# yzqin/s4g-release

Measured on AMD Instinct MI355X. Metric: scenes/sec (25.6k-pt clouds) end-to-end grasp inference, higher is better.
Workload: dtype f32 (f16x2 split)

## Files before the change

include/s4g_ops.h:

```cpp
#ifndef S4G_OPS_H_
#define S4G_OPS_H_

#include <stddef.h>
#include <stdint.h>

#ifdef __cplusplus
extern "C" {
#endif

#define S4G_ABI_VERSION 14


#define S4G_OK 0
#define S4G_EINVAL (-1)
#define S4G_EWORKSPACE (-2)
#define S4G_EUNSUPPORTED (-3)

#define S4G_FLAG_FMAD 1

typedef void *s4g_stream_t;

#define S4G_OP_FPS 1
#define S4G_OP_BALL_QUERY 2
#define S4G_OP_THREE_NN 3
// ... 131 lines not shown
  float *out2;
  int32_t ldc2, split_n;
  float *out_amax2;
  int32_t a_L;
} s4g_gemm_desc_t;

int s4g_mlp_gemm_f32(const s4g_gemm_desc_t *desc, s4g_stream_t stream);

typedef struct s4g_heads_desc {
  int32_t precision, P, N, ldx;
  int32_t C, H0, H1, H2, H3;
  const float *X;
  const void *W_frag[5];
  const float *bias[5];
  const float *w_inv_scale[5];
  float *out[4];
  int32_t channels[4];
  int32_t sigmoid_head;
  const float *a_amax;
  float a_amax_floor;
  int32_t rows_per_scene;
  const void *pre_W_frag[2];
  const float *pre_bias[2];
  const float *pre_w_inv_scale[2];
  const int32_t *pre_nidx;
  const float *pre_nw;
  const float *pre_sparse;
  const float *pre_dense;
  const float *pre_lbias;
  const float *pre_a_amax2;
  int32_t pre_N2;
  int64_t out_batch_stride;
  int32_t head_mask;
} s4g_heads_desc_t;

int s4g_heads_chain_f32(const s4g_heads_desc_t *desc, s4g_stream_t stream);

int s4g_amax_per_scene_f32(const float *x, int64_t B, int64_t n_per_scene, float *out_slots, s4g_stream_t stream);

int s4g_gemm_chain_supported(int loader, int epilogue, int C, int Kpad16);

int s4g_ball_query_i32(const float *xyz_b3n, const float *ctr_b3m, int64_t B,
                       int64_t N, int64_t M, float radius, int64_t K,
                       int32_t *idx_bmk, int32_t *cnt_bm, void *ws,
                       size_t ws_bytes, int flags, s4g_stream_t stream);
int s4g_three_nn_weights_i32(const float *q_b3n1, const float *k_b3n2, int64_t B,
                             int64_t N1, int64_t N2, float eps, int32_t *idx_bn3,
                             float *w_bn3, void *ws, size_t ws_bytes, int flags,
                             s4g_stream_t stream);
size_t s4g_three_nn_grid_workspace_bytes(int64_t B, int64_t N1, int64_t N2);
size_t s4g_three_nn_grid_header_offset(int64_t B, int64_t N2);
int s4g_three_nn_weights_grid_i32(const float *q_b3n1, const float *k_b3n2, int64_t B,
                                  int64_t N1, int64_t N2, float eps, float cell,
                                  int32_t *idx_bn3, float *w_bn3, void *ws,
                                  size_t ws_bytes, int flags, s4g_stream_t stream);

int s4g_three_nn_grid_f32(const float *q_b3n1, const float *k_b3n2, int64_t B, int64_t N1,
                          int64_t N2, float cell, int64_t *idx_bn3, float *d2_bn3, void *ws,
                          size_t ws_bytes, int flags, s4g_stream_t stream);

int s4g_query_group_f32(const float *xyz_b3n, const float *ctr_b3m, int64_t B,
                        int64_t N, int64_t M, float radius, int64_t K,
                        int64_t *idx_bmk, int64_t *cnt_bm, float *grouped_b3mk,
                        void *ws, size_t ws_bytes, int flags, s4g_stream_t stream);

int s4g_group_rel_xyz_i32(const float *xyz_b3n, const float *ctr_b3m, const int32_t *idx_bmk,
// ... 161 lines not shown
```

s4g_release_amd/_cabi.py:

```python
import ctypes
import os

_HERE = os.path.dirname(os.path.abspath(__file__))
LIB_PATH = os.environ.get("S4G_HIP_LIB") or os.path.join(_HERE, "libs4g_hip.so")

S4G_ABI_VERSION = 14
S4G_EINVAL = -1
S4G_EWORKSPACE = -2
S4G_EUNSUPPORTED = -3
S4G_FLAG_FMAD = 1
S4G_OP_FPS, S4G_OP_BALL_QUERY, S4G_OP_THREE_NN = 1, 2, 3

_vp = ctypes.c_void_p
_i64 = ctypes.c_int64
_sz = ctypes.c_size_t
_int = ctypes.c_int
_f32 = ctypes.c_float

_i32 = ctypes.c_int32


class GemmDesc(ctypes.Structure):
    _fields_ = [
        ("loader", _i32), ("epilogue", _i32), ("groups", _i32), ("relu", _i32),
        ("P", _i32), ("Cin", _i32), ("Kpad", _i32), ("Cout", _i32),
        ("W", _vp), ("bias", _vp), ("w_gstride", _i32), ("b_gstride", _i32),
        ("A", _vp), ("lda", _i32), ("a_coff", _i32), ("a_gcol", _i32),
        ("gidx", _vp), ("feat", _vp), ("xyz", _vp), ("ctr", _vp),
        ("Cf", _i32), ("N", _i32), ("M", _i32), ("K", _i32),
        ("nidx", _vp), ("nw", _vp), ("sparse", _vp), ("dense", _vp),
        ("C2", _i32), ("C1", _i32), ("N2", _i32), ("N1", _i32),
        ("out", _vp), ("ldc", _i32), ("c_coff", _i32), ("c_gcol", _i32),
        ("cf_ptr", _vp * 4), ("cf_start", _i32 * 5), ("cf_sigmoid_from", _i32), ("cf_N", _i32),
        ("precision", _i32), ("Kpad16", _i32), ("W_bf16x3", _vp), ("mlp1_w", _vp),
        ("W_f16x2", _vp), ("w_inv_scale", _vp), ("a_amax", _vp), ("a_amax2", _vp),
        ("a_amax_floor", _f32), ("out_amax", _vp), ("W_f16x2_frag", _vp),
        ("W2_f16x2_frag", _vp), ("w2_inv_scale", _vp), ("bias2", _vp), ("Cout2", _i32), ("relu2", _i32),
        ("W3_f16x2_frag", _vp), ("w3_inv_scale", _vp), ("bias3", _vp), ("Cout3", _i32), ("relu3", _i32),
        ("loader_bias", _vp), ("rows_per_scene", _i32), ("rel_xyz4", _vp), ("seg4", _vp), ("seg_rows", _vp),
        ("out2", _vp), ("ldc2", _i32), ("split_n", _i32), ("out_amax2", _vp),
        ("a_L", _i32),
    ]


class HeadsDesc(ctypes.Structure):
    _fields_ = [
        ("precision", _i32), ("P", _i32), ("N", _i32), ("ldx", _i32),
        ("C", _i32), ("H0", _i32), ("H1", _i32), ("H2", _i32), ("H3", _i32),
        ("X", _vp), ("W_frag", _vp * 5), ("bias", _vp * 5), ("w_inv_scale", _vp * 5),
        ("out", _vp * 4), ("channels", _i32 * 4), ("sigmoid_head", _i32),
        ("a_amax", _vp), ("a_amax_floor", _f32), ("rows_per_scene", _i32),
        ("pre_W_frag", _vp * 2), ("pre_bias", _vp * 2), ("pre_w_inv_scale", _vp * 2),
        ("pre_nidx", _vp), ("pre_nw", _vp), ("pre_sparse", _vp), ("pre_dense", _vp),
        ("pre_lbias", _vp), ("pre_a_amax2", _vp), ("pre_N2", _i32), ("out_batch_stride", _i64), ("head_mask", _i32),
    ]


SIGNATURES = {
    "s4g_mlp_gemm_f32": (_int, [ctypes.POINTER(GemmDesc), _vp]),
    "s4g_heads_chain_f32": (_int, [ctypes.POINTER(HeadsDesc), _vp]),
    "s4g_ball_query_i32": (_int, [_vp, _vp, _i64, _i64, _i64, _f32, _i64, _vp, _vp, _vp, _sz,
                                  _int, _vp]),
    "s4g_three_nn_weights_i32": (_int, [_vp, _vp, _i64, _i64, _i64, _f32, _vp, _vp, _vp, _sz,
                                        _int, _vp]),
    "s4g_three_nn_grid_workspace_bytes": (_sz, [_i64, _i64, _i64]),
    "s4g_three_nn_grid_header_offset": (_sz, [_i64, _i64]),
    "s4g_three_nn_weights_grid_i32": (_int, [_vp, _vp, _i64, _i64, _i64, _f32, _f32, _vp, _vp, _vp,
                                             _sz, _int, _vp]),
    "s4g_three_nn_grid_f32": (_int, [_vp, _vp, _i64, _i64, _i64, _f32, _vp, _vp, _vp, _sz, _int, _vp]),
    "s4g_group_points_xyz_f32": (_int, [_vp, _vp, _i64, _i64, _i64, _i64, _vp, _vp, _sz, _vp]),
    "s4g_gemm_chain_supported": (_int, [_int, _int, _int, _int]),
    "s4g_amax_per_scene_f32": (_int, [_vp, _i64, _i64, _vp, _vp]),
    "s4g_interp_add_cl_f32": (_int, [_vp, _vp, _vp, _vp, _vp, _i64, _i64, _i64, _i64, _int, _vp, _vp, _vp]),
    "s4g_group_points_ws_f32": (_int, [_vp, _vp, _i64, _i64, _i64, _i64, _i64, _vp, _vp, _sz, _vp]),
    "s4g_three_interpolate_ws_f32": (_int, [_vp, _vp, _vp, _i64, _i64, _i64, _i64, _vp, _vp, _sz, _int, _vp]),
    "s4g_fps_gather_i32": (_int, [_vp, _i64, _i64, _i64, _vp, _vp, _vp, _sz, _int, _vp]),
    "s4g_fps_prepass_f32": (_int, [_vp, _i64, _i64, _i64, _vp, _vp, _vp]),
    "s4g_fps_gather_ex_i32": (_int, [_vp, _i64, _i64, _i64, _vp, _vp, _vp, _vp, _vp, _sz, _int, _vp]),
    "s4g_fps_prefix_check_f32": (_int, [_vp, _vp, _i64, _i64, _i64, _vp, _int, _vp]),
    "s4g_build_variants": (_int, []),
    "s4g_test_knobs_enabled": (_int, []),
    "s4g_fps_f64": (_int, [_vp, _i64, _i64, _i64, _vp, _vp, _sz, _int, _vp]),
    "s4g_ball_query_f64": (_int, [_vp, _vp, _i64, _i64, _i64, _f32, _i64, _vp, _vp, _int, _vp]),
    "s4g_three_nn_f64": (_int, [_vp, _vp, _i64, _i64, _i64, _vp, _vp, _int, _vp]),
    "s4g_group_points_f64": (_int, [_vp, _vp, _i64, _i64, _i64, _i64, _i64, _vp, _vp]),
    "s4g_group_points_backward_f64": (_int, [_vp, _vp, _i64, _i64, _i64, _i64, _i64, _vp, _vp]),
    "s4g_three_interpolate_f64": (_int, [_vp, _vp, _vp, _i64, _i64, _i64, _i64, _vp, _int, _vp]),
# ... 120 lines not shown
```

s4g_release_amd/csrc/mlp_heads.hip:

```cpp
#include <stdlib.h>

#include "mlp_common.h"

#ifndef S4G_HEADS_ABLATE
#define S4G_HEADS_ABLATE 0
#endif

namespace s4g {

__device__ __forceinline__ void heads_keep_alive(const f32x16& v) { asm volatile("" ::"v"(v)); }

struct HeadsParams {
  int P, N;
  const float* X;
  int ldx;
  const uint16_t* W[5];
  const float* bias[5];
  const float* wsc[5];
  float* out[4];
  int ch[4];
  long long obs[4];
  int head_mask;
  int sigmoid_head;
  const float* a_amax;
  float a_floor;
  int rps;
  const uint16_t* Wp[2];
  const float* bias_p[2];
  const float* wsc_p[2];
  const int* nidx;
  const float* nw;
  const float* sparse;
  const float* dense;
  const float* lbias;
  const float* a_amax2;
  int N2;
};

template <int PL, int HD_RING, int NRBT, bool PRE>
__global__ __launch_bounds__(512, 2) void mlp_heads_kernel(const HeadsParams p) {
  constexpr int BM = 32 * NRBT, C = 256, NW = 8, astr = C + 8, aplane = BM * astr;
  constexpr int FB = PL * 1024;
  extern __shared__ __attribute__((aligned(16))) float smemf[];
  uint16_t* PA = reinterpret_cast<uint16_t*>(smemf);
  uint16_t* PB = PA + PL * aplane;
  float* scr = reinterpret_cast<float*>(PB + PL * aplane);

  const int t = threadIdx.x;
  const int lane = t & 63;
  const int li = lane & 31, lh = lane >> 5;
  const int wv = __builtin_amdgcn_readfirstlane(t >> 6);
  const int p0 = blockIdx.x * BM;
  const uint32_t wf_lane = (uint32_t)lane * 16u;

  float sa = 1.f, inv_sa = 1.f;
  if constexpr (PL == 2) {
    float amax = p.a_floor;
    if constexpr (PRE) {
      if (p.a_amax) amax += amax_rows(p.a_amax, lane, p0, min(p0 + BM, p.P) - 1, p.rps);
      if (p.a_amax2) amax += amax_rows(p.a_amax2, lane, p0, min(p0 + BM, p.P) - 1, p.rps);
    } else if (p.a_amax) {
      amax = fmaxf(amax, amax_rows(p.a_amax, lane, p0, min(p0 + BM, p.P) - 1, p.rps));
    }
    uint32_t ex = __float_as_uint(amax) >> 23;
    ex = ex < 15u ? 15u : (ex > 240u ? 240u : ex);
    ex = __builtin_amdgcn_readfirstlane(ex);
    sa = __uint_as_float((268u - ex) << 23);
    inv_sa = __uint_as_float((ex - 14u) << 23);
  }

  WRef wrs[5];
#pragma unroll
  for (int L = 0; L < 5; ++L) wrs[L] = wref(p.W[L], 0);
  auto woff = [&](int n32, int nks, int ks) { return (size_t)((n32 * nks + ks) * FB); };
  auto w0 = [&](int g, int h) { return wrs[0] + woff(g * 16 + h * 8 + wv, 16, 0); };
  auto w1 = [&](int g, int h) { return wrs[1] + woff(g * 8 + wv, 32, h * 16); };
  auto w2 = [&](int g) { return wrs[2] + woff(g * 8 + wv, 16, 0); };
  auto w3 = [&](int g) { return wrs[3] + woff(g * 4 + (wv & 3), 16, 0); };
  auto wl = [&](int g) { return wrs[4] + woff(g, 8, 0); };
  auto wload = [&](const WRef& w, uint32_t byte_off, int pl) { return wref_load(w, wf_lane + pl * 1024, byte_off); };
  const WRef wp0 = PRE ? wref(p.Wp[0], woff(wv, 16, 0)) : wrs[0];
  const WRef wp1 = PRE ? wref(p.Wp[1], woff(wv, 16, 0)) : wrs[0];

  const int hmask = p.head_mask;
  const int g_first = __builtin_ctz(hmask);
  uint4 ring[HD_RING][PL];
  {
    const WRef w = PRE ? wp0 : w0(g_first, 0);
#pragma unroll
    for (int d = 0; d < HD_RING; ++d)
#pragma unroll
      for (int pl = 0; pl < PL; ++pl) ring[d][pl] = wload(w, d * FB, pl);
  }

#pragma unroll 1
  for (int r0 = 0; r0 < BM; r0 += 64) {
    const int row = r0 + (t >> 3), chunk = t & 7;
    const bool ok = p0 + row < p.P;
    float4 ra[8];
    if constexpr (PRE) {
      const int pos = ok ? p0 + row : 0;
      const int bq = pos / p.N;
      int i3[3];
      float w3[3];
#pragma unroll
      for (int k = 0; k < 3; ++k) {
        i3[k] = bq * p.N2 + p.nidx[(size_t)pos * 3 + k];
        w3[k] = p.nw[(size_t)pos * 3 + k];
      }
#pragma unroll
      for (int h = 0; h < 2; ++h) {
        float4 a[4], b[4], c[4], y[4], bb[4];
#pragma unroll
        for (int kk = 0; kk < 4; ++kk) {
          const int col = (h * 4 + kk) * 32 + chunk * 4;
          a[kk] = *reinterpret_cast<const float4*>(p.sparse + (size_t)i3[0] * 256 + col);
          b[kk] = *reinterpret_cast<const float4*>(p.sparse + (size_t)i3[1] * 256 + col);
          c[kk] = *reinterpret_cast<const float4*>(p.sparse + (size_t)i3[2] * 256 + col);
          bb[kk] = *reinterpret_cast<const float4*>(p.lbias + col);
          y[kk] = p.dense ? *reinterpret_cast<const float4*>(p.dense + (size_t)pos * 256 + col)
                          : make_float4(0.f, 0.f, 0.f, 0.f);
        }
#pragma unroll
        for (int kk = 0; kk < 4; ++kk) {
          const float av[4] = {a[kk].x, a[kk].y, a[kk].z, a[kk].w}, bv[4] = {b[kk].x, b[kk].y, b[kk].z, b[kk].w};
          const float cv[4] = {c[kk].x, c[kk].y, c[kk].z, c[kk].w}, yv[4] = {y[kk].x, y[kk].y, y[kk].z, y[kk].w};
          const float bi[4] = {bb[kk].x, bb[kk].y, bb[kk].z, bb[kk].w};
          float r[4];
#pragma unroll
          for (int e = 0; e < 4; ++e) {
            float acc = __fmul_rn(av[e], w3[0]);
            acc = __fadd_rn(acc, __fmul_rn(bv[e], w3[1]));
            acc = __fadd_rn(acc, __fmul_rn(cv[e], w3[2]));
            r[e] = ok ? fmaxf(__fadd_rn(__fadd_rn(yv[e], acc), bi[e]), 0.f) : 0.f;
          }
          ra[h * 4 + kk] = make_float4(r[0], r[1], r[2], r[3]);
        }
      }
    } else {
    const float* src = p.X + (size_t)(ok ? p0 + row : 0) * p.ldx + chunk * 4;
#pragma unroll
    for (int kt = 0; kt < 8; ++kt)
      ra[kt] = ok ? nt_load4(src + kt * 32) : make_float4(0.f, 0.f, 0.f, 0.f);
    }
#pragma unroll
    for (int kt = 0; kt < 8; ++kt) {
      uint16_t* dst = PA + row * astr + kt * 32 + chunk * 4;
      if constexpr (PL == 2) {
        uint2 h, l;
        split2_h<false>(ra[kt], sa, h, l);
        *reinterpret_cast<uint2*>(dst) = h;
        *reinterpret_cast<uint2*>(dst + aplane) = l;
      } else {
        *reinterpret_cast<uint2*>(dst) = make_uint2(cvt_pk_bf16(ra[kt].x, ra[kt].y), cvt_pk_bf16(ra[kt].z, ra[kt].w));
      }
    }
  }
  __syncthreads();

#define S4G_HD_TERM(NRB, PA_, PB_, ZERO)                                                            \
  _Pragma("unroll") for (int rb = 0; rb < NRB; ++rb)                                                \
    acc[rb] = chain_mfma<PL>(bf[PB_], af[rb][PA_], (ZERO) ? zero16 : acc[rb]);
#define S4G_HD_STRIP(PANEL, NRB, ROWOFF, WCUR, NKS, WNEXT)                                          \
  {                                                                                                 \
    const uint16_t* a_lane = (PANEL) + ((ROWOFF) + li) * astr + 8 * lh;                             \
    uint4 afn[NRBT][PL];                                                                            \
    _Pragma("unroll") for (int rb = 0; rb < NRB; ++rb) _Pragma("unroll") for (int pl = 0; pl < PL; ++pl) \
      afn[rb][pl] = *reinterpret_cast<const uint4*>(a_lane + pl * aplane + rb * 32 * astr);         \
    const WRef wcur_ = (WCUR);                                                                      \
    const WRef wnext_ = (WNEXT);                                                                    \
    _Pragma("unroll") for (int ks = 0; ks < NKS; ++ks) {                                            \
      const int d = ks % HD_RING;                                                                   \
      const int ksn = ks + 1 == NKS ? 0 : ks + 1;                                                   \
      uint4 af[NRBT][PL], bf[PL];                                                                   \
      _Pragma("unroll") for (int rb = 0; rb < NRB; ++rb) _Pragma("unroll") for (int pl = 0; pl < PL; ++pl) { \
        af[rb][pl] = afn[rb][pl];                                                                   \
        if (!(S4G_HEADS_ABLATE & 2))                                                                \
          afn[rb][pl] = *reinterpret_cast<const uint4*>(a_lane + pl * aplane + rb * 32 * astr + ksn * 16); \
      }                                                                                             \
      _Pragma("unroll") for (int pl = 0; pl < PL; ++pl) bf[pl] = ring[d][pl];                       \
      {                                                                                             \
        const int kr = ks + HD_RING;                                                                \
        _Pragma("unroll") for (int pl = 0; pl < PL; ++pl)                                           \
          if (!(S4G_HEADS_ABLATE & 1))                                                              \
            ring[d][pl] = kr < NKS ? wload(wcur_, kr * FB, pl) : wload(wnext_, (kr - NKS) * FB, pl); \
      }                                                                                             \
      if constexpr (PL == 2) {                                                                      \
        S4G_HD_TERM(NRB, 0, 1, ks == 0)                                                             \
        S4G_HD_TERM(NRB, 1, 0, false)                                                               \
        S4G_HD_TERM(NRB, 0, 0, false)                                                               \
      } else {                                                                                      \
        S4G_HD_TERM(NRB, 0, 0, ks == 0)                                                             \
      }                                                                                             \
      _Pragma("unroll") for (int q = 0; q < PL; ++q) {                                              \
        __builtin_amdgcn_sched_group_barrier(0x008, 1, 0);                                          \
        __builtin_amdgcn_sched_group_barrier(0x020, 1, 0);                                          \
        __builtin_amdgcn_sched_group_barrier(0x008, 1, 0);                                          \
        __builtin_amdgcn_sched_group_barrier(0x100, 1, 0);                                          \
      }                                                                                             \
      __builtin_amdgcn_sched_barrier(0);                                                            \
    }                                                                                               \
  }

  f32x16 zero16;
#pragma unroll
  for (int r = 0; r < 16; ++r) zero16[r] = 0.f;
  f32x16 acc[NRBT];
  float* epi_s = scr + wv * 64;

  auto stage_sb2 = [&](const float* wsc, const float* bias, int gch, float mul) {
    epi_s[lane] = lane < 32 ? (PL == 2 ? mul * wsc[gch + lane] : 1.f) : bias[gch + lane - 32];
  };
  auto stage_sb = [&](int L, int gch, float mul) { stage_sb2(p.wsc[L], p.bias[L], gch, mul); };

  float inv_sh = 1.f;
  auto panel_epilogue_to = [&](uint16_t* PD, auto nrb_tag, int rowoff, int pch0) {
    constexpr int NRB = decltype(nrb_tag)::value;
    if (S4G_HEADS_ABLATE & 4) {
#pragma unroll
      for (int rb = 0; rb < NRB; ++rb) heads_keep_alive(acc[rb]);
      if (!(S4G_HEADS_ABLATE & 8)) {
        __syncthreads();
        __syncthreads();
      }
      return;
    }
    float tmax = 0.f;
#pragma unroll
    for (int j = 0; j < 4; ++j) {
      const float4 sc4 = *reinterpret_cast<const float4*>(epi_s + 8 * j + 4 * lh);
      const float4 b4 = *reinterpret_cast<const float4*>(epi_s + 32 + 8 * j + 4 * lh);
      const float scv[4] = {sc4.x, sc4.y, sc4.z, sc4.w};
      const float bv[4] = {b4.x, b4.y, b4.z, b4.w};
#pragma unroll
      for (int rb = 0; rb < NRB; ++rb) {
        const f32x2 x01 = pk_fma(f32x2{acc[rb][4 * j], acc[rb][4 * j + 1]}, f32x2{scv[0], scv[1]}, f32x2{bv[0], bv[1]});
        const f32x2 x23 = pk_fma(f32x2{acc[rb][4 * j + 2], acc[rb][4 * j + 3]}, f32x2{scv[2], scv[3]}, f32x2{bv[2], bv[3]});
        const float x[4] = {fmaxf(x01.x, 0.f), fmaxf(x01.y, 0.f), fmaxf(x23.x, 0.f), fmaxf(x23.y, 0.f)};
#pragma unroll
        for (int e = 0; e < 4; ++e) acc[rb][4 * j + e] = x[e];
        if constexpr (PL == 2) {
          tmax = fmaxf(fmaxf(tmax, x[0]), x[1]);
          tmax = fmaxf(fmaxf(tmax, x[2]), x[3]);
        }
      }
    }
    float sh = 1.f;
    if constexpr (PL == 2) {
      const uint32_t wm = wave_max_u32(__float_as_uint(tmax));
      if (lane == 0) scr[NW * 64 + wv] = __uint_as_float(wm);
    }
    __syncthreads();
    if constexpr (PL == 2) {
      float hmax = scr[NW * 64];
#pragma unroll
      for (int w = 1; w < NW; ++w) hmax = fmaxf(hmax, scr[NW * 64 + w]);
      uint32_t exh = __float_as_uint(hmax) >> 23;
      exh = exh < 15u ? 15u : (exh > 240u ? 240u : exh);
      exh = __builtin_amdgcn_readfirstlane(exh);
      sh = __uint_as_float((268u - exh) << 23);
      inv_sh = __uint_as_float((exh - 14u) << 23);
    }
#pragma unroll
    for (int j = 0; j < 4; ++j)
#pragma unroll
      for (int rb = 0; rb < NRB; ++rb) {
        uint16_t* dst = PD + (rowoff + rb * 32 + li) * astr + pch0 + 8 * j + 4 * lh;
        if constexpr (PL == 2) {
          const float4 v = make_float4(acc[rb][4 * j], acc[rb][4 * j + 1], acc[rb][4 * j + 2], acc[rb][4 * j + 3]);
          uint2 h, l;
          split2_h<false>(v, sh, h, l);
          *reinterpret_cast<uint2*>(dst) = h;
          *reinterpret_cast<uint2*>(dst + aplane) = l;
        } else {
          *reinterpret_cast<uint2*>(dst) = make_uint2(cvt_pk_bf16(acc[rb][4 * j], acc[rb][4 * j + 1]),
                                                      cvt_pk_bf16(acc[rb][4 * j + 2], acc[rb][4 * j + 3]));
        }
      }
    __syncthreads();
  };
  auto panel_epilogue = [&](auto nrb_tag, int rowoff, int pch0) { panel_epilogue_to(PB, nrb_tag, rowoff, pch0); };
  using full = std::integral_constant<int, NRBT>;
  using half = std::integral_constant<int, NRBT / 2>;

  if constexpr (PRE) {
    stage_sb2(p.wsc_p[0], p.bias_p[0], wv * 32, inv_sa);
    S4G_HD_STRIP(PA, NRBT, 0, wp0, 16, wp1)
    panel_epilogue(full{}, 0, wv * 32);
    stage_sb2(p.wsc_p[1], p.bias_p[1], wv * 32, inv_sh);
    S4G_HD_STRIP(PB, NRBT, 0, wp1, 16, w0(g_first, 0))
    panel_epilogue_to(PA, full{}, 0, wv * 32);
    inv_sa = inv_sh;
  }

  for (int g = g_first, gn; g >= 0; g = gn) {
    const int rest = hmask >> (g + 1);
    gn = rest ? g + 1 + __builtin_ctz(rest) : -1;
    const int gnx = gn >= 0 ? gn : g;
    f32x16 acc1[NRBT];
    stage_sb(0, g * 512 + wv * 32, inv_sa);
    S4G_HD_STRIP(PA, NRBT, 0, w0(g, 0), 16, w1(g, 0))
    panel_epilogue(full{}, 0, wv * 32);
    S4G_HD_STRIP(PB, NRBT, 0, w1(g, 0), 16, w0(g, 1))
#pragma unroll
    for (int rb = 0; rb < NRBT; ++rb)
#pragma unroll
      for (int r = 0; r < 16; r += 2) {
        const f32x2 v = f32x2{acc[rb][r], acc[rb][r + 1]} * f32x2{inv_sh, inv_sh};
        acc1[rb][r] = v.x;
        acc1[rb][r + 1] = v.y;
      }
    stage_sb(0, g * 512 + 256 + wv * 32, inv_sa);
    S4G_HD_STRIP(PA, NRBT, 0, w0(g, 1), 16, w1(g, 1))
    panel_epilogue(full{}, 0, wv * 32);
    S4G_HD_STRIP(PB, NRBT, 0, w1(g, 1), 16, w2(g))
#pragma unroll
    for (int rb = 0; rb < NRBT; ++rb)
#pragma unroll
      for (int r = 0; r < 16; r += 2) {
        const f32x2 v = pk_fma(f32x2{acc[rb][r], acc[rb][r + 1]}, f32x2{inv_sh, inv_sh}, f32x2{acc1[rb][r], acc1[rb][r + 1]});
        acc[rb][r] = v.x;
        acc[rb][r + 1] = v.y;
      }
    stage_sb(1, g * 256 + wv * 32, 1.f);
    panel_epilogue(full{}, 0, wv * 32);
    stage_sb(2, g * 256 + wv * 32, inv_sh);
    S4G_HD_STRIP(PB, NRBT, 0, w2(g), 16, w3(g))
    panel_epilogue(full{}, 0, wv * 32);
    {
      const int row3 = (wv >> 2) * (BM / 2), cg = wv & 3;
      stage_sb(3, g * 128 + cg * 32, inv_sh);
      const WRef after = wv < NRBT ? wl(g) : w0(gnx, 0);
      S4G_HD_STRIP(PB, NRBT / 2, row3, w3(g), 16, after)
      panel_epilogue(half{}, row3, cg * 32);
    }
    if (wv < NRBT) {
      stage_sb(4, g * 32, inv_sh);
      S4G_HD_STRIP(PB, 1, wv * 32, wl(g), 8, w0(gnx, 0))
      const int row = p0 + wv * 32 + li;
      const int b = row / p.N, pt = row - b * p.N;
      const int nch = p.ch[g];
      float* __restrict__ base = p.out[g] + (size_t)b * (size_t)p.obs[g] + pt;
#pragma unroll
      for (int j = 0; j < 4; ++j) {
        const float4 sc4 = *reinterpret_cast<const float4*>(epi_s + 8 * j + 4 * lh);
        const float4 b4 = *reinterpret_cast<const float4*>(epi_s + 32 + 8 * j + 4 * lh);
        const float scv[4] = {sc4.x, sc4.y, sc4.z, sc4.w};
        const float bv[4] = {b4.x, b4.y, b4.z, b4.w};
#pragma unroll
        for (int e = 0; e < 4; ++e) {
          const int c = 8 * j + 4 * lh + e;
          float x = __fmaf_rn(acc[0][4 * j + e], scv[e], bv[e]);
          if (g == p.sigmoid_head) x = 1.0f / (1.0f + expf(-x));
          if (c < nch && row < p.P) base[(size_t)c * p.N] = x;
        }
      }
    }
  }
#undef S4G_HD_STRIP
#undef S4G_HD_TERM
}

template <int PL, int HD_RING, int NRBT, bool PRE>
static int launch_heads_cfg(const HeadsParams& p, hipStream_t st) {
  constexpr int BM = 32 * NRBT;
  constexpr size_t lds = sizeof(uint16_t) * 2 * PL * BM * (256 + 8) + sizeof(float) * (8 * 64 + 16);
  static_assert(lds <= 160 * 1024, "one workgroup's panels must fit a CU's LDS");
  static LdsAttrCache lds_cache;
  if (int rc = allow_dynamic_lds(reinterpret_cast<const void*>(&mlp_heads_kernel<PL, HD_RING, NRBT, PRE>), lds, lds_cache)) return rc;
  hipLaunchKernelGGL((mlp_heads_kernel<PL, HD_RING, NRBT, PRE>), dim3((unsigned)((p.P + BM - 1) / BM)), dim3(512), lds, st, p);
  S4G_LAUNCH_CHECK();
  return S4G_OK;
}
template <int PL, int HD_RING, int NRBT>
static int launch_heads(const HeadsParams& p, hipStream_t st) {
  return p.Wp[0] ? launch_heads_cfg<PL, HD_RING, NRBT, true>(p, st) : launch_heads_cfg<PL, HD_RING, NRBT, false>(p, st);
}

}

extern "C" int s4g_heads_chain_f32(const s4g_heads_desc_t* d, s4g_stream_t stream) {
  using namespace s4g;
  if (!d || d->P < 0 || d->N <= 0) return S4G_EINVAL;
  const bool pre = d->pre_W_frag[0] != nullptr;
  if (!pre && (!d->X || (d->ldx & 3) || d->ldx < 256 || ((uintptr_t)d->X & 15))) return S4G_EINVAL;
  if (pre && (!d->pre_W_frag[1] || !d->pre_bias[0] || !d->pre_bias[1] || !d->pre_nidx || !d->pre_nw ||
              !d->pre_sparse || !d->pre_lbias || d->pre_N2 < 3 || ((uintptr_t)d->pre_sparse & 15) ||
              ((uintptr_t)d->pre_dense & 15) || ((uintptr_t)d->pre_lbias & 15) ||
              (d->precision == S4G_GEMM_F16X2 && (!d->pre_w_inv_scale[0] || !d->pre_w_inv_scale[1]))))
    return S4G_EINVAL;
  if (d->precision != S4G_GEMM_F16X2 && d->precision != S4G_GEMM_BF16) return S4G_EINVAL;
  if (d->C != 256 || d->H0 != 512 || d->H1 != 256 || d->H2 != 256 || d->H3 != 128) return S4G_EUNSUPPORTED;
  HeadsParams p;
  p.P = d->P;
  p.N = d->N;
  p.X = d->X;
  p.ldx = d->ldx;
  for (int l = 0; l < 5; ++l) {
    if (!d->W_frag[l] || !d->bias[l] || (d->precision == S4G_GEMM_F16X2 && !d->w_inv_scale[l])) return S4G_EINVAL;
    p.W[l] = (const uint16_t*)d->W_frag[l];
    p.bias[l] = d->bias[l];
    p.wsc[l] = d->w_inv_scale[l];
  }
  p.head_mask = d->head_mask ? d->head_mask : 15;
  if (p.head_mask < 0 || p.head_mask > 15) return S4G_EINVAL;
  for (int h = 0; h < 4; ++h) {
    p.out[h] = nullptr;
    p.ch[h] = 0;
    p.obs[h] = 0;
    if (!((p.head_mask >> h) & 1)) continue;
    if (!d->out[h] || d->channels[h] <= 0 || d->channels[h] > 32) return S4G_EINVAL;
    p.out[h] = d->out[h];
    p.ch[h] = d->channels[h];
    if (d->out_batch_stride != 0 && d->out_batch_stride < (int64_t)d->channels[h] * d->N) return S4G_EINVAL;
    p.obs[h] = d->out_batch_stride != 0 ? (long long)d->out_batch_stride : (long long)d->channels[h] * d->N;
  }
  p.sigmoid_head = d->sigmoid_head;
  p.a_amax = d->a_amax;
  p.a_floor = d->a_amax_floor;
  p.rps = d->rows_per_scene > 0 ? d->rows_per_scene : 0;
  for (int l = 0; l < 2; ++l) {
    p.Wp[l] = pre ? (const uint16_t*)d->pre_W_frag[l] : nullptr;
    p.bias_p[l] = pre ? d->pre_bias[l] : nullptr;
    p.wsc_p[l] = pre ? d->pre_w_inv_scale[l] : nullptr;
  }
  p.nidx = pre ? d->pre_nidx : nullptr;
  p.nw = pre ? d->pre_nw : nullptr;
  p.sparse = pre ? d->pre_sparse : nullptr;
  p.dense = pre ? d->pre_dense : nullptr;
  p.lbias = pre ? d->pre_lbias : nullptr;
  p.a_amax2 = pre ? d->pre_a_amax2 : nullptr;
  p.N2 = pre ? d->pre_N2 : 0;
  if (d->precision == S4G_GEMM_F16X2 && !d->a_amax && !(d->a_amax_floor > 0.f)) return S4G_EINVAL;
  if (d->P == 0) return S4G_OK;
  hipStream_t st = (hipStream_t)stream;
  if (d->precision == S4G_GEMM_F16X2) return launch_heads<2, 4, 2>(p, st);
  return launch_heads<1, 4, 4>(p, st);
}
```

s4g_release_amd/fused.py:

```python
import ctypes
import os

import torch

from . import _cabi
from . import functions as _F

_i32 = ctypes.c_int32
_fp = ctypes.c_void_p
GemmDesc = _cabi.GemmDesc
HeadsDesc = _cabi.HeadsDesc

LOAD_PLAIN, LOAD_GATHER, LOAD_INTERP, LOAD_GATHER_MLP1, LOAD_GATHER_ADD, LOAD_INTERP_ADD = 0, 1, 2, 3, 4, 5
EPI_STORE, EPI_MAX, EPI_CF = 0, 1, 2

NETWORK_KINDS = {(9, 4): "PN2_CLS", (6, 3): "PN2"}
HEADS_CLS = ("score", "frame_R", "frame_t", "movable_logits")
HEADS_CONTACT = ("scene_score_logits", "frame_R", "frame_t", "movable_logits")
CONTACT_RAW_CHANNELS = (3, 6, 3, 5)
CONTACT_OUT_CHANNELS = (3, 9, 3, 5)


def fold_conv_bn(block):
    w = block.conv.weight.detach().double().flatten(1)
# ... 283 lines not shown
        d.precision = {"fp32": 0, "bf16x3": 1, "bf16": 2, "f16x2": 3}[self.precision]
        d.Kpad16, d.W_bf16x3 = layer.kpad16, layer.W3.data_ptr()
        d.W_f16x2, d.w_inv_scale = layer.Wh2.data_ptr(), layer.w_inv_scale.data_ptr()
        bf16 = self.precision == "bf16"
        frag = (lambda l: l.Wfrag_bf16) if bf16 else (lambda l: l.Wfrag)
        if layer.Wfrag is not None:
            d.W_f16x2_frag = frag(layer).data_ptr()
        for k, v in kw.items():
            if isinstance(v, torch.Tensor):
                v = v.data_ptr()
            if v is not None:
                setattr(d, k, v)
        flops = 2.0 * P * layer.cout * layer.cin * layer.groups
        if layer2 is not None:
            d.W2_f16x2_frag = frag(layer2).data_ptr()
            d.w2_inv_scale, d.bias2 = layer2.w_inv_scale.data_ptr(), layer2.bias.data_ptr()
            d.Cout2, d.relu2 = layer2.cout, int(relu2)
            flops += 2.0 * P * layer2.cout * layer2.cin * layer2.groups
            name = "%s+%s" % (name, name2 or name[:-1] + str(int(name[-1]) + 1))
        if layer3 is not None:
            d.W3_f16x2_frag = frag(layer3).data_ptr()
            d.w3_inv_scale, d.bias3 = layer3.w_inv_scale.data_ptr(), layer3.bias.data_ptr()
            d.Cout3, d.relu3 = layer3.cout, 1
            flops += 2.0 * P * layer3.cout * layer3.cin * layer3.groups
            name += "+" + name3
        if rows_used is not None:
            per_row = flops / P
            flops = lambda: per_row * float(rows_used.sum().item())
        with _F._timed("gemm[%s P=%d K=%d N=%dx%d]" % (name, P, layer.cin, layer.groups, layer.cout),
                       0, flops):
            rc = _cabi.lib().s4g_mlp_gemm_f32(ctypes.byref(d), _F._stream())
        _cabi.check(rc, "mlp_gemm " + name)

    def _heads(self, x, x_amax, outs, B, N0, pre=None, head_mask=0):
        d = HeadsDesc()
        bf16 = self.precision == "bf16"
        d.precision = 2 if bf16 else 3
        d.P, d.N = B * N0, N0
        d.C, d.H0, d.H1, d.H2, d.H3 = 256, 512, 256, 256, 128
        flops = 0.0
        name = "heads.0-3+logits"
        if pre is None:
            d.X, d.ldx = x.data_ptr(), x.shape[1]
        else:
            frag = (lambda l: l.Wfrag_bf16) if bf16 else (lambda l: l.Wfrag)
            for i, layer in enumerate(pre["layers"]):
                d.pre_W_frag[i] = frag(layer).data_ptr()
                d.pre_bias[i] = layer.bias.data_ptr()
                d.pre_w_inv_scale[i] = layer.w_inv_scale.data_ptr()
                flops += 2.0 * B * N0 * layer.cout * layer.cin
            d.pre_nidx, d.pre_nw = pre["nidx"].data_ptr(), pre["nw"].data_ptr()
            d.pre_sparse, d.pre_N2 = pre["sparse"].data_ptr(), pre["N2"]
            d.pre_dense = None if pre["dense"] is None else pre["dense"].data_ptr()
            d.pre_lbias = pre["loader_bias"].data_ptr()
            d.pre_a_amax2 = None if pre["a_amax2"] is None else pre["a_amax2"].data_ptr()
            x_amax = pre["a_amax"]
            name = "%s+%s" % (pre["name"], name)
        nrun = len([h for h in range(4) if (head_mask or 15) >> h & 1])
        for l, layer in enumerate(self.heads_fused):
            d.W_frag[l] = (layer.Wfrag_bf16 if bf16 else layer.Wfrag).data_ptr()
            d.bias[l] = layer.bias.data_ptr()
            d.w_inv_scale[l] = layer.w_inv_scale.data_ptr()
            if l < 4:
                flops += 2.0 * B * N0 * layer.cout * layer.cin * layer.groups * nrun / 4.0
        flops += 2.0 * B * N0 * sum(c for h, c in enumerate(self.head_channels) if (head_mask or 15) >> h & 1) * 128
        d.head_mask = head_mask
        run = [h for h in range(4) if (head_mask or 15) >> h & 1]
        for h, o in enumerate(outs):
            d.channels[h] = self.head_channels[h]
            if h not in run:
                continue
            d.out[h] = o.data_ptr()
            if o.stride(0) != self.head_channels[h] * N0:
                d.out_batch_stride = o.stride(0)
        d.sigmoid_head = 3
        d.a_amax = None if x_amax is None else x_amax.data_ptr()
        d.a_amax_floor = 0.0 if pre is None else pre["a_amax_floor"]
        d.rows_per_scene = N0
        if head_mask not in (0, 15):
            name += "[heads %s]" % "".join(str(h) for h in range(4) if head_mask >> h & 1)
        with _F._timed("gemm[%s P=%d K=256 N=%dx(512,256,256,128,c)]" % (name, B * N0, nrun), 0, flops):
            rc = _cabi.lib().s4g_heads_chain_f32(ctypes.byref(d), _F._stream())
        _cabi.check(rc, "heads_chain")

    def _fps_gather(self, xyz, M, want_dist=False, run=None):
        B, _, N = xyz.shape
        idx = torch.empty((B, M), dtype=torch.int32, device=xyz.device)
        ctr = torch.empty((B, 3, M), dtype=torch.float32, device=xyz.device)
        ws, nbytes = _F._workspace(_cabi.S4G_OP_FPS, xyz.device, B, N, M, 0)
        dist = torch.empty((B, M), dtype=torch.float32, device=xyz.device) if want_dist else None
        with _F._timed("fps[N=%d,M=%d]" % (N, M), B * (12 * N + 8 * M)):
            if dist is not None or run is not None:
                rc = _cabi.lib().s4g_fps_gather_ex_i32(xyz.data_ptr(), B, N, M, idx.data_ptr(), ctr.data_ptr(),
                                                       None if dist is None else dist.data_ptr(),
                                                       None if run is None else run.data_ptr(),
                                                       _F._ptr(ws), nbytes, _F._DIST_FLAGS, _F._stream())
                if rc == _cabi.S4G_EUNSUPPORTED and run is None:
                    dist, rc = None, 0
                    rc = _cabi.lib().s4g_fps_gather_i32(xyz.data_ptr(), B, N, M, idx.data_ptr(), ctr.data_ptr(),
                                                        _F._ptr(ws), nbytes, _F._DIST_FLAGS, _F._stream())
            else:
                rc = _cabi.lib().s4g_fps_gather_i32(xyz.data_ptr(), B, N, M, idx.data_ptr(),
                                                    ctr.data_ptr(), _F._ptr(ws), nbytes,
                                                    _F._DIST_FLAGS, _F._stream())
        _cabi.check(rc, "fps_gather")
        return (idx, ctr, dist) if want_dist else (idx, ctr)

    def _fps_prefix_check(self, ctr, dist, M2):
# ... 543 lines not shown
```

Measured before the change: 2033.

## Use 96-row heads tiles with low-half input spilled to global workspace

Adds a three-row-block (96-row) f16x2 heads kernel variant that keeps only half of the low-precision input plane in LDS and spills the low half of the input panel to a global workspace. Tiles are assigned per scene, the first layer is split into two accumulator strips, and the low half is reloaded from the workspace between heads. The aim is larger tiles per workgroup at the same LDS budget, giving more weight reuse per row. The cost is extra global stores and reloads, added schedule complexity, and a new workspace that has to be passed through the ABI.

```diff
diff --git a/include/s4g_ops.h b/include/s4g_ops.h
--- a/include/s4g_ops.h
+++ b/include/s4g_ops.h
@@ -187,6 +187,8 @@
   int32_t pre_N2;
   int64_t out_batch_stride;
   int32_t head_mask;
+  void *x_lo_workspace;
+  uint64_t x_lo_workspace_bytes;
 } s4g_heads_desc_t;
 
 int s4g_heads_chain_f32(const s4g_heads_desc_t *desc, s4g_stream_t stream);
diff --git a/s4g_release_amd/_cabi.py b/s4g_release_amd/_cabi.py
--- a/s4g_release_amd/_cabi.py
+++ b/s4g_release_amd/_cabi.py
@@ -53,6 +53,7 @@
         ("pre_W_frag", _vp * 2), ("pre_bias", _vp * 2), ("pre_w_inv_scale", _vp * 2),
         ("pre_nidx", _vp), ("pre_nw", _vp), ("pre_sparse", _vp), ("pre_dense", _vp),
         ("pre_lbias", _vp), ("pre_a_amax2", _vp), ("pre_N2", _i32), ("out_batch_stride", _i64), ("head_mask", _i32),
+        ("x_lo_workspace", _vp), ("x_lo_workspace_bytes", ctypes.c_uint64),
     ]
 
 
diff --git a/s4g_release_amd/csrc/mlp_heads.hip b/s4g_release_amd/csrc/mlp_heads.hip
--- a/s4g_release_amd/csrc/mlp_heads.hip
+++ b/s4g_release_amd/csrc/mlp_heads.hip
@@ -25,6 +25,7 @@
   const float* a_amax;
   float a_floor;
   int rps;
+  uint16_t* xlo;
   const uint16_t* Wp[2];
   const float* bias_p[2];
   const float* wsc_p[2];
@@ -41,26 +42,46 @@
 __global__ __launch_bounds__(512, 2) void mlp_heads_kernel(const HeadsParams p) {
   constexpr int BM = 32 * NRBT, C = 256, NW = 8, astr = C + 8, aplane = BM * astr;
   constexpr int FB = PL * 1024;
+  constexpr bool XW = PL == 2 && NRBT == 3;
+  constexpr int PLA = XW ? 1 : PL;
+  static_assert(NRBT == 2 || NRBT == 4 || XW, "three position blocks: the f16x2 form only");
   extern __shared__ __attribute__((aligned(16))) float smemf[];
   uint16_t* PA = reinterpret_cast<uint16_t*>(smemf);
-  uint16_t* PB = PA + PL * aplane;
+  uint16_t* PB = PA + PLA * aplane;
   float* scr = reinterpret_cast<float*>(PB + PL * aplane);
 
   const int t = threadIdx.x;
   const int lane = t & 63;
   const int li = lane & 31, lh = lane >> 5;
   const int wv = __builtin_amdgcn_readfirstlane(t >> 6);
-  const int p0 = blockIdx.x * BM;
+  int p0, nvalid, scene = 0, tile = 0;
+  if constexpr (XW) {
+    const int tps = (p.N + BM - 1) / BM;
+    scene = (int)blockIdx.x / tps;
+    tile = (int)blockIdx.x - scene * tps;
+    p0 = scene * p.N + tile * BM;
+    nvalid = min(BM, min(p.N, p.P - scene * p.N) - tile * BM);
+    if (nvalid <= 0) return;
+  } else {
+    p0 = blockIdx.x * BM;
+    nvalid = min(BM, p.P - p0);
+  }
+  auto xlo_off = [&](int r, int c) { return (c >> 7) * aplane + r * astr + 128 + (c & 127); };
+  const WRef xws = XW ? wref(p.xlo + (size_t)p0 * C, 0) : WRef{};
+  auto xws_store = [&](uint2 v, uint32_t lane_off, uint32_t byte_off) {
+    typedef unsigned int u32x2 __attribute__((ext_vector_type(2)));
+    __builtin_amdgcn_raw_buffer_store_b64(u32x2{v.x, v.y}, xws.r, (int)lane_off, (int)byte_off, 0);
+  };
   const uint32_t wf_lane = (uint32_t)lane * 16u;
 
   float sa = 1.f, inv_sa = 1.f;
   if constexpr (PL == 2) {
     float amax = p.a_floor;
     if constexpr (PRE) {
-      if (p.a_amax) amax += amax_rows(p.a_amax, lane, p0, min(p0 + BM, p.P) - 1, p.rps);
-      if (p.a_amax2) amax += amax_rows(p.a_amax2, lane, p0, min(p0 + BM, p.P) - 1, p.rps);
+      if (p.a_amax) amax += amax_rows(p.a_amax, lane, p0, p0 + nvalid - 1, p.rps);
+      if (p.a_amax2) amax += amax_rows(p.a_amax2, lane, p0, p0 + nvalid - 1, p.rps);
     } else if (p.a_amax) {
-      amax = fmaxf(amax, amax_rows(p.a_amax, lane, p0, min(p0 + BM, p.P) - 1, p.rps));
+      amax = fmaxf(amax, amax_rows(p.a_amax, lane, p0, p0 + nvalid - 1, p.rps));
     }
     uint32_t ex = __float_as_uint(amax) >> 23;
     ex = ex < 15u ? 15u : (ex > 240u ? 240u : ex);
@@ -96,7 +117,8 @@
 #pragma unroll 1
   for (int r0 = 0; r0 < BM; r0 += 64) {
     const int row = r0 + (t >> 3), chunk = t & 7;
-    const bool ok = p0 + row < p.P;
+    if (BM % 64 != 0 && row >= BM) break;
+    const bool ok = row < nvalid;
     float4 ra[8];
     if constexpr (PRE) {
       const int pos = ok ? p0 + row : 0;
@@ -150,7 +172,12 @@
         uint2 h, l;
         split2_h<false>(ra[kt], sa, h, l);
         *reinterpret_cast<uint2*>(dst) = h;
-        *reinterpret_cast<uint2*>(dst + aplane) = l;
+        if constexpr (XW) {
+          *reinterpret_cast<uint2*>(PB + xlo_off(row, kt * 32 + chunk * 4)) = l;
+          if (!PRE && ok) xws_store(l, (uint32_t)(row * C + chunk * 4) * 2u, kt * 64);
+        } else {
+          *reinterpret_cast<uint2*>(dst + aplane) = l;
+        }
       } else {
         *reinterpret_cast<uint2*>(dst) = make_uint2(cvt_pk_bf16(ra[kt].x, ra[kt].y), cvt_pk_bf16(ra[kt].z, ra[kt].w));
       }
@@ -158,15 +185,17 @@
   }
   __syncthreads();
 
-#define S4G_HD_TERM(NRB, PA_, PB_, ZERO)                                                            \
+#define S4G_HD_TERM(ACC, NRB, PA_, PB_, ZERO)                                                       \
   _Pragma("unroll") for (int rb = 0; rb < NRB; ++rb)                                                \
-    acc[rb] = chain_mfma<PL>(bf[PB_], af[rb][PA_], (ZERO) ? zero16 : acc[rb]);
-#define S4G_HD_STRIP(PANEL, NRB, ROWOFF, WCUR, NKS, WNEXT)                                          \
+    ACC[rb] = chain_mfma<PL>(bf[PB_], af[rb][PA_], (ZERO) ? zero16 : ACC[rb]);
+#define S4G_HD_KOFF(XF, PL_, KS) ((XF) && (PL_) == 1 ? ((KS) >> 3) * aplane + ((KS) & 7) * 16 : (KS) * 16)
+#define S4G_HD_STRIP_X(ACC, XF, PANEL, NRB, ROWOFF, WCUR, NKS, WNEXT)                               \
   {                                                                                                 \
     const uint16_t* a_lane = (PANEL) + ((ROWOFF) + li) * astr + 8 * lh;                             \
+    const uint16_t* a_low = (XF) ? PB + ((ROWOFF) + li) * astr + 8 * lh + 128 : a_lane + aplane;    \
     uint4 afn[NRBT][PL];                                                                            \
     _Pragma("unroll") for (int rb = 0; rb < NRB; ++rb) _Pragma("unroll") for (int pl = 0; pl < PL; ++pl) \
-      afn[rb][pl] = *reinterpret_cast<const uint4*>(a_lane + pl * aplane + rb * 32 * astr);         \
+      afn[rb][pl] = *reinterpret_cast<const uint4*>((pl ? a_low : a_lane) + rb * 32 * astr);        \
     const WRef wcur_ = (WCUR);                                                                      \
     const WRef wnext_ = (WNEXT);                                                                    \
     _Pragma("unroll") for (int ks = 0; ks < NKS; ++ks) {                                            \
@@ -176,7 +205,7 @@
       _Pragma("unroll") for (int rb = 0; rb < NRB; ++rb) _Pragma("unroll") for (int pl = 0; pl < PL; ++pl) { \
         af[rb][pl] = afn[rb][pl];                                                                   \
         if (!(S4G_HEADS_ABLATE & 2))                                                                \
-          afn[rb][pl] = *reinterpret_cast<const uint4*>(a_lane + pl * aplane + rb * 32 * astr + ksn * 16); \
+          afn[rb][pl] = *reinterpret_cast<const uint4*>((pl ? a_low : a_lane) + rb * 32 * astr + S4G_HD_KOFF(XF, pl, ksn)); \
       }                                                                                             \
       _Pragma("unroll") for (int pl = 0; pl < PL; ++pl) bf[pl] = ring[d][pl];                       \
       {                                                                                             \
@@ -186,11 +215,11 @@
             ring[d][pl] = kr < NKS ? wload(wcur_, kr * FB, pl) : wload(wnext_, (kr - NKS) * FB, pl); \
       }                                                                                             \
       if constexpr (PL == 2) {                                                                      \
-        S4G_HD_TERM(NRB, 0, 1, ks == 0)                                                             \
-        S4G_HD_TERM(NRB, 1, 0, false)                                                               \
-        S4G_HD_TERM(NRB, 0, 0, false)                                                               \
+        S4G_HD_TERM(ACC, NRB, 0, 1, ks == 0)                                                        \
+        S4G_HD_TERM(ACC, NRB, 1, 0, false)                                                          \
+        S4G_HD_TERM(ACC, NRB, 0, 0, false)                                                          \
       } else {                                                                                      \
-        S4G_HD_TERM(NRB, 0, 0, ks == 0)                                                             \
+        S4G_HD_TERM(ACC, NRB, 0, 0, ks == 0)                                                        \
       }                                                                                             \
       _Pragma("unroll") for (int q = 0; q < PL; ++q) {                                              \
         __builtin_amdgcn_sched_group_barrier(0x008, 1, 0);                                          \
@@ -198,9 +227,16 @@
         __builtin_amdgcn_sched_group_barrier(0x008, 1, 0);                                          \
         __builtin_amdgcn_sched_group_barrier(0x100, 1, 0);                                          \
       }                                                                                             \
+      if constexpr ((NRB) == 3) {           \
+        _Pragma("unroll") for (int q = 0; q < 4; ++q) {                                             \
+          __builtin_amdgcn_sched_group_barrier(0x008, 1, 0);                                        \
+          __builtin_amdgcn_sched_group_barrier(0x100, 1, 0);                                        \
+        }                                                                                           \
+      }                                                                                             \
       __builtin_amdgcn_sched_barrier(0);                                                            \
     }                                                                                               \
   }
+#define S4G_HD_STRIP(PANEL, NRB, ROWOFF, WCUR, NKS, WNEXT) S4G_HD_STRIP_X(acc, false, PANEL, NRB, ROWOFF, WCUR, NKS, WNEXT)
 
   f32x16 zero16;
 #pragma unroll
@@ -214,8 +250,9 @@
   auto stage_sb = [&](int L, int gch, float mul) { stage_sb2(p.wsc[L], p.bias[L], gch, mul); };
 
   float inv_sh = 1.f;
-  auto panel_epilogue_to = [&](uint16_t* PD, auto nrb_tag, int rowoff, int pch0) {
+  auto panel_epilogue_on = [&](auto& acc, uint16_t* PD, auto xd_tag, auto nrb_tag, int rowoff, int pch0) {
     constexpr int NRB = decltype(nrb_tag)::value;
+    constexpr bool XD = decltype(xd_tag)::value;
     if (S4G_HEADS_ABLATE & 4) {
 #pragma unroll
       for (int rb = 0; rb < NRB; ++rb) heads_keep_alive(acc[rb]);
@@ -271,13 +308,22 @@
           uint2 h, l;
           split2_h<false>(v, sh, h, l);
           *reinterpret_cast<uint2*>(dst) = h;
-          *reinterpret_cast<uint2*>(dst + aplane) = l;
+          if constexpr (XD) {
+            const int r = rowoff + rb * 32 + li, c = pch0 + 8 * j + 4 * lh;
+            *reinterpret_cast<uint2*>(PB + xlo_off(r, c)) = l;
+            if (r < nvalid) xws_store(l, (uint32_t)(li * C + 4 * lh) * 2u, (uint32_t)((rowoff + rb * 32) * C + pch0 + 8 * j) * 2u);
+          } else {
+            *reinterpret_cast<uint2*>(dst + aplane) = l;
+          }
         } else {
           *reinterpret_cast<uint2*>(dst) = make_uint2(cvt_pk_bf16(acc[rb][4 * j], acc[rb][4 * j + 1]),
                                                       cvt_pk_bf16(acc[rb][4 * j + 2], acc[rb][4 * j + 3]));
         }
       }
     __syncthreads();
+  };
+  auto panel_epilogue_to = [&](uint16_t* PD, auto nrb_tag, int rowoff, int pch0) {
+    panel_epilogue_on(acc, PD, std::false_type{}, nrb_tag, rowoff, pch0);
   };
   auto panel_epilogue = [&](auto nrb_tag, int rowoff, int pch0) { panel_epilogue_to(PB, nrb_tag, rowoff, pch0); };
   using full = std::integral_constant<int, NRBT>;
@@ -285,13 +331,101 @@
 
   if constexpr (PRE) {
     stage_sb2(p.wsc_p[0], p.bias_p[0], wv * 32, inv_sa);
-    S4G_HD_STRIP(PA, NRBT, 0, wp0, 16, wp1)
+    S4G_HD_STRIP_X(acc, XW, PA, NRBT, 0, wp0, 16, wp1)
     panel_epilogue(full{}, 0, wv * 32);
     stage_sb2(p.wsc_p[1], p.bias_p[1], wv * 32, inv_sh);
     S4G_HD_STRIP(PB, NRBT, 0, wp1, 16, w0(g_first, 0))
-    panel_epilogue_to(PA, full{}, 0, wv * 32);
+    panel_epilogue_on(acc, PA, std::bool_constant<XW>{}, full{}, 0, wv * 32);
     inv_sa = inv_sh;
   }
+
+  if constexpr (XW) {
+    for (int g = g_first, gn; g >= 0; g = gn) {
+      const int rest = hmask >> (g + 1);
+      gn = rest ? g + 1 + __builtin_ctz(rest) : -1;
+      const int gnx = gn >= 0 ? gn : g;
+      f32x16 accb[NRBT];
+      S4G_HD_STRIP_X(acc, true, PA, NRBT, 0, w0(g, 0), 16, w0(g, 1))
+      S4G_HD_STRIP_X(accb, true, PA, NRBT, 0, w0(g, 1), 16, w1(g, 0))
+      stage_sb(0, g * 512 + wv * 32, inv_sa);
+      panel_epilogue(full{}, 0, wv * 32);
+      S4G_HD_STRIP(PB, NRBT, 0, w1(g, 0), 16, w1(g, 1))
+#pragma unroll
+      for (int rb = 0; rb < NRBT; ++rb)
+#pragma unroll
+        for (int r = 0; r < 16; r += 2) {
+          const f32x2 v = f32x2{acc[rb][r], acc[rb][r + 1]} * f32x2{inv_sh, inv_sh};
+          acc[rb][r] = v.x;
+          acc[rb][r + 1] = v.y;
+        }
+      stage_sb(0, g * 512 + 256 + wv * 32, inv_sa);
+      panel_epilogue_on(accb, PB, std::false_type{}, full{}, 0, wv * 32);
+      S4G_HD_STRIP_X(accb, false, PB, NRBT, 0, w1(g, 1), 16, w2(g))
+#pragma unroll
+      for (int rb = 0; rb < NRBT; ++rb)
+#pragma unroll
+        for (int r = 0; r < 16; r += 2) {
+          const f32x2 v = pk_fma(f32x2{accb[rb][r], accb[rb][r + 1]}, f32x2{inv_sh, inv_sh}, f32x2{acc[rb][r], acc[rb][r + 1]});
+          acc[rb][r] = v.x;
+          acc[rb][r + 1] = v.y;
+        }
+      stage_sb(1, g * 256 + wv * 32, 1.f);
+      panel_epilogue(full{}, 0, wv * 32);
+      stage_sb(2, g * 256 + wv * 32, inv_sh);
+      S4G_HD_STRIP(PB, NRBT, 0, w2(g), 16, w3(g))
+      panel_epilogue(full{}, 0, wv * 32);
+      {
+        const int cg = wv & 3;
+        stage_sb(3, g * 128 + cg * 32, inv_sh);
+        const WRef after = wv < NRBT ? wl(g) : w0(gnx, 0);
+        if (wv < 4) {
+          S4G_HD_STRIP(PB, 2, 0, w3(g), 16, after)
+          panel_epilogue(std::integral_constant<int, 2>{}, 0, cg * 32);
+        } else {
+          S4G_HD_STRIP(PB, 1, 64, w3(g), 16, after)
+          panel_epilogue(std::integral_constant<int, 1>{}, 64, cg * 32);
+        }
+      }
+      if (wv < NRBT) {
+        stage_sb(4, g * 32, inv_sh);
+        S4G_HD_STRIP(PB, 1, wv * 32, wl(g), 8, w0(gnx, 0))
+        const int lrow = wv * 32 + li;
+        const int nch = p.ch[g];
+        const WRef ob = wref(p.out[g] + (size_t)scene * (size_t)p.obs[g] + tile * BM, 0);
+        const uint32_t o_lane = (uint32_t)(lrow + 4 * lh * p.N) * 4u;
+#pragma unroll
+        for (int j = 0; j < 4; ++j) {
+          const float4 sc4 = *reinterpret_cast<const float4*>(epi_s + 8 * j + 4 * lh);
+          const float4 b4 = *reinterpret_cast<const float4*>(epi_s + 32 + 8 * j + 4 * lh);
+          const float scv[4] = {sc4.x, sc4.y, sc4.z, sc4.w};
+          const float bv[4] = {b4.x, b4.y, b4.z, b4.w};
+#pragma unroll
+          for (int e = 0; e < 4; ++e) {
+            const int c = 8 * j + 4 * lh + e;
+            float x = __fmaf_rn(acc[0][4 * j + e], scv[e], bv[e]);
+            if (g == p.sigmoid_head) x = 1.0f / (1.0f + expf(-x));
+            if (c < nch && lrow < nvalid)
+              __builtin_amdgcn_raw_buffer_store_b32(__float_as_uint(x), ob.r, (int)o_lane, (int)((uint32_t)((8 * j + e) * p.N) * 4u), 0);
+          }
+        }
+      } else if (gn >= 0) {
+        constexpr int NPC = BM * 32, NTH = (NW - NRBT) * 64, NIT = (NPC + NTH - 1) / NTH;
+        static_assert(NTH % 32 == 0, "a thread keeps its column piece from round to round");
+        const int i0 = (wv - NRBT) * 64 + lane, r0 = i0 >> 5;
+        uint16_t* dst0 = PB + xlo_off(r0, (i0 & 31) * 8);
+        uint4 v[NIT];
+#pragma unroll
+        for (int i = 0; i < NIT; ++i) {
+          v[i] = make_uint4(0u, 0u, 0u, 0u);
+          if (r0 < nvalid - i * (NTH / 32)) v[i] = wref_load(xws, (uint32_t)i0 * 16u, i * NTH * 16);
+        }
+#pragma unroll
+        for (int i = 0; i < NIT; ++i)
+          if (r0 < BM - i * (NTH / 32)) *reinterpret_cast<uint4*>(dst0 + i * (NTH / 32) * astr) = v[i];
+      }
+      if (gn >= 0) __syncthreads();
+    }
+  } else
 
   for (int g = g_first, gn; g >= 0; g = gn) {
     const int rest = hmask >> (g + 1);
@@ -358,17 +492,21 @@
     }
   }
 #undef S4G_HD_STRIP
+#undef S4G_HD_STRIP_X
+#undef S4G_HD_KOFF
 #undef S4G_HD_TERM
 }
 
 template <int PL, int HD_RING, int NRBT, bool PRE>
 static int launch_heads_cfg(const HeadsParams& p, hipStream_t st) {
   constexpr int BM = 32 * NRBT;
-  constexpr size_t lds = sizeof(uint16_t) * 2 * PL * BM * (256 + 8) + sizeof(float) * (8 * 64 + 16);
+  constexpr int planes = PL == 2 && NRBT == 3 ? 3 : 2 * PL;
+  constexpr size_t lds = sizeof(uint16_t) * planes * BM * (256 + 8) + sizeof(float) * (8 * 64 + 16);
   static_assert(lds <= 160 * 1024, "one workgroup's panels must fit a CU's LDS");
   static LdsAttrCache lds_cache;
   if (int rc = allow_dynamic_lds(reinterpret_cast<const void*>(&mlp_heads_kernel<PL, HD_RING, NRBT, PRE>), lds, lds_cache)) return rc;
-  hipLaunchKernelGGL((mlp_heads_kernel<PL, HD_RING, NRBT, PRE>), dim3((unsigned)((p.P + BM - 1) / BM)), dim3(512), lds, st, p);
+  const long long tiles = PL == 2 && NRBT == 3 ? (long long)((p.P + p.N - 1) / p.N) * ((p.N + BM - 1) / BM) : (p.P + BM - 1) / BM;
+  hipLaunchKernelGGL((mlp_heads_kernel<PL, HD_RING, NRBT, PRE>), dim3((unsigned)tiles), dim3(512), lds, st, p);
   S4G_LAUNCH_CHECK();
   return S4G_OK;
 }
@@ -419,6 +557,8 @@
   p.a_amax = d->a_amax;
   p.a_floor = d->a_amax_floor;
   p.rps = d->rows_per_scene > 0 ? d->rows_per_scene : 0;
+  p.xlo = (uint16_t*)d->x_lo_workspace;
+  if (p.xlo && (((uintptr_t)p.xlo & 15) || d->x_lo_workspace_bytes < (uint64_t)d->P * 256 * sizeof(uint16_t))) return S4G_EINVAL;
   for (int l = 0; l < 2; ++l) {
     p.Wp[l] = pre ? (const uint16_t*)d->pre_W_frag[l] : nullptr;
     p.bias_p[l] = pre ? d->pre_bias[l] : nullptr;
@@ -434,6 +574,7 @@
   if (d->precision == S4G_GEMM_F16X2 && !d->a_amax && !(d->a_amax_floor > 0.f)) return S4G_EINVAL;
   if (d->P == 0) return S4G_OK;
   hipStream_t st = (hipStream_t)stream;
+  if (d->precision == S4G_GEMM_F16X2 && p.xlo && p.N <= (1 << 22)) return launch_heads<2, 4, 3>(p, st);
   if (d->precision == S4G_GEMM_F16X2) return launch_heads<2, 4, 2>(p, st);
   return launch_heads<1, 4, 4>(p, st);
 }
diff --git a/s4g_release_amd/fused.py b/s4g_release_amd/fused.py
--- a/s4g_release_amd/fused.py
+++ b/s4g_release_amd/fused.py
@@ -339,6 +339,14 @@
             rc = _cabi.lib().s4g_mlp_gemm_f32(ctypes.byref(d), _F._stream())
         _cabi.check(rc, "mlp_gemm " + name)
 
+    def _x_lo_workspace(self, dev, P):
+        cache = self.__dict__.setdefault("_x_lo_ws", {})
+        key = (str(dev), int(P), _F._stream())
+        ws = cache.get(key)
+        if ws is None:
+            ws = cache[key] = torch.empty((P, 256), dtype=torch.float16, device=dev)
+        return ws
+
     def _heads(self, x, x_amax, outs, B, N0, pre=None, head_mask=0):
         d = HeadsDesc()
         bf16 = self.precision == "bf16"
@@ -381,6 +389,9 @@
             if o.stride(0) != self.head_channels[h] * N0:
                 d.out_batch_stride = o.stride(0)
         d.sigmoid_head = 3
+        if not bf16:
+            ws = self._x_lo_workspace(outs[run[0]].device, B * N0)
+            d.x_lo_workspace, d.x_lo_workspace_bytes = ws.data_ptr(), ws.numel() * ws.element_size()
         d.a_amax = None if x_amax is None else x_amax.data_ptr()
         d.a_amax_floor = 0.0 if pre is None else pre["a_amax_floor"]
         d.rows_per_scene = N0
```

Result: no change. 2051, median of 6 (+0.9%).
